# LauraBaracaldo/LauraBaracaldo-Spatial-Meta-Kriging-for-Distributed-Inference-for-Binary-Response

Measured on AMD Instinct MI355X. Metric: MCMC iters/sec (all subsets, whole node) + end-to-end wall-clock, n=500k K=250, higher is better.
Workload: dtype f64

## Files before the change

### laurabaracaldo-spatial-meta-kriging-for-distributed-inference-for-binary-response_amd/csrc/mk_gemm.hpp

```cpp
#pragma once
#include "mk_common.hpp"

namespace mk {

typedef double d4 __attribute__((ext_vector_type(4)));
typedef double d2 __attribute__((ext_vector_type(2)));

constexpr int GB_K = 16;
__host__ __device__ constexpr int gb_stride(int len) {
  return len == 256 ? 272 : (len == 128 ? 144 : (len == 64 ? 80 : 48));
}
__host__ __device__ constexpr int gb_img(int len) { return GB_K * gb_stride(len); }
__host__ __device__ constexpr int gb_lds_bytes(int tm, int tn) { return 2 * (gb_img(tm) + gb_img(tn)) * 8; }
static_assert(gb_lds_bytes(128, 128) == MK_GD_LDS_BYTES, "mk_common.hpp LDS size");
static_assert(128 * GB_K <= gb_img(128) && 64 * GB_K <= gb_img(64) && 32 * GB_K <= gb_img(32),
              "k-contiguous images fit their slots");

template <int BM, int BN>
struct AccT {
  d4 v[BM][BN];
};
typedef AccT<4, 4> Acc;

template <int BM, int BN>
// ... 258 lines not shown
  for (int w = 0; w < 4; ++w) {
    if (syrk_rb(w, 0) != w || syrk_cb(w, SYRK_SLOTS - 1) != 7 - w) return false;
    for (int s = 4; s < SYRK_SLOTS; ++s)
      if (syrk_rb(w, s) != 7 - w) return false;
  }
  return true;
}
static_assert(syrk_rows_static(), "slot 0 / slots 4.. have the same row choice on every wave");

struct AccSyrk {
  d4 v[SYRK_SLOTS];
};
__device__ inline int syrk_wave() { return __builtin_amdgcn_readfirstlane((int)(threadIdx.x >> 6)); }
__device__ inline int syrk_row(int w, int s) { return 16 * syrk_rb(w, s) + (threadIdx.x & 15); }
__device__ inline int syrk_col(int w, int s, int r) { return 16 * syrk_cb(w, s) + ((threadIdx.x & 63) >> 4) + 4 * r; }

__device__ inline void mma_chunk_syrk(const double* Ps, AccSyrk& acc, int w) {
  constexpr int LD = gb_stride(128);
  const int lane = threadIdx.x & 63;
  const int li = lane & 15, lk = lane >> 4;
#pragma unroll
  for (int ks = 0; ks < GB_K / 4; ++ks) {
    const double* row = Ps + (ks * 4 + lk) * LD + li;
    const double p0 = row[16 * w], p1 = row[16 * (7 - w)];
    const double y0 = -p0, y1 = -p1;
    double xb[SYRK_SLOTS];
#pragma unroll
    for (int s = 0; s < SYRK_SLOTS - 1; ++s) xb[s] = row[16 * syrk_cb(w, s)];
    xb[SYRK_SLOTS - 1] = p1;
#pragma unroll
    for (int s = 0; s < SYRK_SLOTS; ++s) {
      const double ya = s == 0 ? y0 : (s >= 4 ? y1 : (s <= w ? y0 : y1));
      acc.v[s] = __builtin_amdgcn_mfma_f64_16x16x4f64(xb[s], ya, acc.v[s], 0, 0, 0);
    }
  }
}

__device__ inline void gemm_syrk_128(const double* __restrict__ P, long s, int K, AccSyrk& acc, double* lds) {
  constexpr int STAGE = gb_img(128);
  if (K <= 0) return;
  const int nch = K / GB_K;
  const int w = syrk_wave();
  dma_chunk<true, 128>(P, s, 0, lds);
  asm volatile("s_waitcnt vmcnt(0)" ::: "memory");
  __syncthreads();
  for (int c = 0; c < nch; ++c) {
    if (c + 1 < nch) dma_chunk<true, 128>(P, s, GB_K * (c + 1), lds + ((c + 1) & 1) * STAGE);
    mma_chunk_syrk(lds + (c & 1) * STAGE, acc, w);
    asm volatile("s_waitcnt vmcnt(0)" ::: "memory");
    __syncthreads();
  }
}

__device__ inline void acc_load_syrk(AccSyrk& acc, const double* C, long ldc) {
  const int w = syrk_wave();
#pragma unroll
  for (int s = 0; s < SYRK_SLOTS; ++s)
#pragma unroll
    for (int r = 0; r < 4; ++r) acc.v[s][r] = C[syrk_row(w, s) + (long)syrk_col(w, s, r) * ldc];
}
__device__ inline void store_tile_syrk(double* C, long ldc, const AccSyrk& acc) {
  const int w = syrk_wave();
#pragma unroll
  for (int s = 0; s < SYRK_SLOTS; ++s)
#pragma unroll
    for (int r = 0; r < 4; ++r) C[syrk_row(w, s) + (long)syrk_col(w, s, r) * ldc] = acc.v[s][r];
}
__device__ inline void store_tile_syrk_lds(double* T, int tld, const AccSyrk& acc) {
  const int w = syrk_wave();
#pragma unroll
  for (int s = 0; s < SYRK_SLOTS; ++s)
#pragma unroll
    for (int r = 0; r < 4; ++r) {
      const int rr = syrk_row(w, s), cc = syrk_col(w, s, r);
      T[rr + cc * tld] = rr >= cc ? acc.v[s][r] : 0.0;
    }
  const int zr = threadIdx.x & 15, zc = threadIdx.x >> 4;
#pragma unroll
  for (int rb = 0; rb < 8; ++rb)
#pragma unroll
    for (int cb = rb + 1; cb < 8; ++cb) T[(16 * rb + zr) + (16 * cb + zc) * tld] = 0.0;
}

}
```

### laurabaracaldo-spatial-meta-kriging-for-distributed-inference-for-binary-response_amd/csrc/mk_kernels.hpp

```cpp
#pragma once
#include "mk_types.hpp"
#include "mk_corr.hpp"

namespace mk {
inline int xcd_grid_h(int S, int T) { return 8 * ((S + 7) / 8) * T; }
template <int MODEL>
__global__ void k_cov_candidate(Model md, MatSet ms, int h0, int hc, int which, int iter, const int* slist, const int* scount);
typedef void (*CovCandidateKernel)(Model, MatSet, int, int, int, int, const int*, const int*);
inline CovCandidateKernel cov_candidate_kernel(int model) {
  return model == MK_COV_EXPONENTIAL ? k_cov_candidate<MK_COV_EXPONENTIAL> : k_cov_candidate<MK_COV_MATERN>;
}
template <int TM, int TN = TM>
__global__ void k_chol_update(MatSet ms, int S, int h0, int hc, int k, int ia, int ib, int j0, int j1,
                              const int* slist, const int* scount, int syrk);
template <int TM>
__global__ void k_chol_trsm(MatSet ms, int S, int h0, int hc, int k, int ia, int ib, const int* slist,
                            const int* scount);
int pv_grid(int max_entries, int nt, int ntt);
template <int TM>
__global__ void k_chol_update_trsm(MatSet ms, int S, int h0, int hc, int k, int ia, int ib, int j0, int extra,
                                   const int* slist, const int* scount, int syrk);
__global__ void k_chol_diag(MatSet ms, const int* n_s, int h0, int hc, int k, double* ld_part, double* quad_c, int* info,
                            const int* slist, const int* scount, int cj0, int cj1, int syrk);
__global__ void k_inv_copydiag(MatSet ms, const int* list, const int* count);
template <int TM>
__global__ void k_inv_level(MatSet ms, const int* list, const int* count, int sz, int phase);
__global__ void k_lauum(MatSet ms, const int* n_s, const int* list, const int* count);
__global__ void k_qblocks(MatSet ms, const int* n_s, const int* list, const int* count);
__global__ void k_take_border(Model md, MatSet ms, const int* list, const int* count, const double* zc);
__global__ void k_cand_border(Model md, MatSet ms, int h0, int hc);
__global__ void k_pred_draw_runs(Model md, const double* kz, const double* kA, int k_lo, const int* plist,
                                 const int* pcount, const int* run_start, int j_end);
__global__ void k_run_start(const int* plist, const int* pcount, int* run_start, int j);
__global__ void k_border_step(Model md, MatSet ms, int k);
__global__ void k_nu_border(Model md, MatSet ms);
__global__ void k_border_quad(Model md);
__global__ void k_trmv_Z(Model md, MatSet ms);
template <int MODEL>
__global__ void k_pred_PT(Model md, const int* list, const int* count);
__global__ void k_pred_PT_matern(Model md, const int* list, const int* count);
__global__ void k_matern_table(Model md, int h0, int hc, int which, int iter, const int* slist, const int* scount);
__global__ void k_matern_table_list(Model md, const int* list, const int* count);
typedef void (*PredPTKernel)(Model, const int*, const int*);
inline PredPTKernel pred_PT_kernel(int model) {
  return model == MK_COV_EXPONENTIAL ? k_pred_PT<MK_COV_EXPONENTIAL> : k_pred_PT<MK_COV_MATERN>;
}
template <bool GEN>
__global__ void k_pred_var(Model md, MatSet ms, const int* list, const int* count);
__global__ void k_pred_var_reduce(Model md, int nt, const int* list, const int* count);
__global__ void k_beta(Model md, int iter);
__global__ void k_Aphase(Model md, int iter);
__global__ void k_theta_mh(Model md, MatSet ms, int h0, int hc, int which, int iter);
__global__ void k_dirty_list(Model md, int force, int* list_inv, int* count_inv, int* list_pred, int* count_pred);
template <int Q>
__global__ void k_sweep(Model md, MatSet ms, int iter, const int* adm, int* fb);
template <int Q>
__global__ void k_sweep_mg(Model md, MatSet ms, int iter, double* part, int* cnt, int* xcc, int* err, int* adm, int spins_max);
template <int Q, int KR, int P, int HH, int LN>
__global__ void k_sweep_site(Model md, MatSet ms, int iter);
inline size_t sweep_site_lds_bytes(int ns_max, int q, int lean = 0) { return (size_t)ns_max * q * (lean ? 4 : 3) * 8 + (size_t)ns_max * 4; }
inline const void* sweep_site_kernel(int q, int kr, int lean = 1) {
  if (q == 1) {
    if (kr == 1)
      return lean == 1 ? (const void*)k_sweep_site<1, 4, 2, 0, 1> : (const void*)k_sweep_site<1, 4, 2, 0, 2>;
    return lean == 1 ? (const void*)k_sweep_site<1, 8, 2, 0, 1> : (const void*)k_sweep_site<1, 8, 2, 0, 2>;
  }
  switch (q) {
    case 2: return kr == 1 ? (const void*)k_sweep_site<2, 4, 1, 0, 0> : (const void*)k_sweep_site<2, 8, 1, 0, 0>;
    case 3: return kr == 1 ? (const void*)k_sweep_site<3, 4, 1, 0, 0> : nullptr;
    default: return nullptr;
  }
}
template <int Q>
__global__ void k_sweep_step(Model md, MatSet ms, int iter, int B, double* part);
inline const void* sweep_step_kernel(int q) {
  switch (q) {
    case 1: return (const void*)k_sweep_step<1>;
    case 2: return (const void*)k_sweep_step<2>;
    case 3: return (const void*)k_sweep_step<3>;
    default: return (const void*)k_sweep_step<4>;
  }
}
inline const void* sweep_kernel(int q, bool mg) {
  switch (q) {
    case 1: return mg ? (const void*)k_sweep_mg<1> : (const void*)k_sweep<1>;
    case 2: return mg ? (const void*)k_sweep_mg<2> : (const void*)k_sweep<2>;
    case 3: return mg ? (const void*)k_sweep_mg<3> : (const void*)k_sweep<3>;
    default: return mg ? (const void*)k_sweep_mg<4> : (const void*)k_sweep<4>;
  }
}
__global__ void k_record(Model md, int iter);
__global__ void k_record_w(Model md, int iter);
__global__ void k_adapt(Model md, int b);
__global__ void k_pred_draw(Model md, int iter, int kidx);
__global__ void k_quantiles(const double* data, long subset_stride, long row_stride, int n_rows, int n_cols,
                            const double* probs, int n_probs, double* out);
__global__ void k_quantiles_prob(const double* data, long subset_stride, long row_stride, int n_rows, int n_cols,
                                 const double* probs, int n_probs, double* out, ProbSrc ps);
__global__ void k_pred_prob(const double* w, long row_stride, int n_rows, int n_cols, double* out, ProbSrc ps);
__global__ void k_chain_diag(const double* data, long subset_stride, long row_stride, int n_rows, int n_cols, double* out);
__global__ void k_chain_diag_prob(const double* data, long subset_stride, long row_stride, int n_rows, int n_cols,
                                  double* out, ProbSrc ps);
__global__ void k_diag_worst(const double* d, int S, long C, double* out);
__global__ void k_combine(const double* grids, int K, long G, double* out, int mean);
__global__ void k_record_kept(Model md, int kidx);
__global__ void k_kept_dirty(Model md, const double* th_prev, int* slist, int* scount, int* plist, int* pcount);
__global__ void k_flip_pairs(MatSet ms, const int* plist, const int* pcount);
__global__ void k_kept_phi(Model md, const double* th, int n, double* phis);
__global__ void k_krig_g(Model md, MatSet ms, const double* z, double* Gt, int j, int nkp);
// ... 21 lines not shown
```

### laurabaracaldo-spatial-meta-kriging-for-distributed-inference-for-binary-response_amd/csrc/mk_linalg.hip

```cpp
#include "mk_gemm.hpp"
#include "mk_types.hpp"
#include "mk_corr.hpp"

namespace mk {

__device__ inline void candidate_theta(const Model& md, int s, int h, int which, int iter, double* phi, double* nu) {
  const Key key = subset_key(md, s);
  const double* th = md.theta + (long)s * md.n_theta;
  const int idx_phi = md.ntri + h, idx_nu = md.ntri + md.q + h;
  double tphi = th[idx_phi];
  double tnu = (md.cov_model == MK_COV_MATERN) ? th[idx_nu] : 0.0;
  if (which == 0 || which == 1) {
    const int j_mh = (which == 0) ? md.o_phi + h : md.o_nu + h;
    const double z = proposal_normal(key, (uint32_t)j_mh, (uint32_t)iter);
    const double step = exp(md.tune[(long)s * md.n_mh_max + j_mh]) * z;
    if (which == 0) tphi += step; else tnu += step;
  }
  *phi = logit_inv(tphi, md.phi_a[h], md.phi_b[h]);
  *nu = (md.cov_model == MK_COV_MATERN) ? logit_inv(tnu, md.nu_a[h], md.nu_b[h]) : 0.0;
}

struct CandGen {
  const double* cx;
  const double* cy;
// ... 744 lines not shown
  if (cj1 > cj0 && syrk) {
    AccSyrk a;
    acc_load_syrk(a, Mt, ld);
    gemm_syrk_128(M + base + (long)cj0 * MK_NB * ld, ld, (cj1 - cj0) * MK_NB, a, sm);
    store_tile_syrk_lds(T, TLD, a);
  } else if (cj1 > cj0) {
    Acc acc;
    acc_load(acc, Mt, ld);
    const long jo = (long)cj0 * MK_NB * ld;
    gemm_tile<128, 128, true, true, true>(M + base + jo, ld, M + base + jo, ld, (cj1 - cj0) * MK_NB,
                                          (cj1 - cj0) * MK_NB, acc, sm);
#pragma unroll
    for (int bm = 0; bm < 4; ++bm)
#pragma unroll
      for (int bn = 0; bn < 4; ++bn)
#pragma unroll
        for (int r = 0; r < 4; ++r) {
          const int rr = acc_row<128>(bm), cc = acc_col<128>(bn, r);
          T[rr + cc * TLD] = rr >= cc ? acc.v[bm][bn][r] : 0.0;
        }
  } else {
    constexpr int NL = MK_NB * MK_NB / (256 * 2);
    d2 v[NL];
#pragma unroll
    for (int j = 0; j < NL; ++j) {
      const int e = 2 * (tid + 256 * j);
      v[j] = *reinterpret_cast<const d2*>(Mt + (e & 127) + (long)(e >> 7) * ld);
    }
#pragma unroll
    for (int j = 0; j < NL; ++j) {
      const int e = 2 * (tid + 256 * j);
      const int r = e & 127, c = e >> 7;
      T[r + c * TLD] = (r >= c) ? v[j].x : 0.0;
      T[r + 1 + c * TLD] = (r + 1 >= c) ? v[j].y : 0.0;
    }
  }
  __syncthreads();
  MK_TSTAMP(40);
  bool bad = false;
  double* W = winv_slot(ms, sh, slot, k);
  factor_invert_tile(T, dg, xd, Sb, ns - base, quad_c + sh, &bad);
  if (tid < 64) {
    double v = 0.0;
    for (int r = tid; r < MK_NB; r += 64) v += (base + r < ns) ? 2.0 * log(dg[r]) : 0.0;
#pragma unroll
    for (int o = 32; o > 0; o >>= 1) v += __shfl_xor(v, o, 64);
    if (tid == 0) {
      ld_part[(long)sh * ms.nt + k] = v;
      if (bad) info[sh] = 1;
    }
  }
  MK_TSTAMP(41);
  store_tile_lw(T, dg, xd, Mt, ld, W);
  MK_TSTAMP(42);
}

#ifndef MK_TRI_SKIP
#define MK_TRI_SKIP 1
#endif
__device__ inline double* wmat(const MatSet& ms, int sh) { return ms.W + (long)sh * mat_elems(ms); }

__global__ __launch_bounds__(256) void k_inv_copydiag(MatSet ms, const int* __restrict__ list, const int* __restrict__ count) {
  const int part = blockIdx.x % MK_CD_SPLIT, rest = blockIdx.x / MK_CD_SPLIT;
  const int e = rest / ms.nt, k = rest % ms.nt;
  if (e >= *count) return;
  const int sh = list[e];
  const double* Wd = winv_slot(ms, sh, ms.cur[sh], k);
  const long ld = ms.ld;
  double* Wt = wmat(ms, sh) + k * MK_NB + (long)k * MK_NB * ld;
  constexpr int PER = MK_NB * MK_NB / MK_CD_SPLIT;
  const int e0 = part * PER;
  d2 v[PER / 512];
#pragma unroll
  for (int j = 0; j < PER / 512; ++j) v[j] = *reinterpret_cast<const d2*>(Wd + e0 + 2 * (threadIdx.x + 256 * j));
#pragma unroll
  for (int j = 0; j < PER / 512; ++j) {
    const int e2 = e0 + 2 * (threadIdx.x + 256 * j);
    *reinterpret_cast<d2*>(Wt + (e2 & 127) + (long)(e2 >> 7) * ld) = v[j];
  }
}

template <int TM>
__global__ __launch_bounds__(256, 2) void k_inv_level(MatSet ms, const int* __restrict__ list,
                                                      const int* __restrict__ count, int sz, int phase) {
  extern __shared__ __attribute__((aligned(16))) double lds[];
  constexpr int SUBR = MK_NB / TM, SUB = SUBR * SUBR;
  const int npairs = (ms.nt + 2 * sz - 1) / (2 * sz);
  const int per = npairs * sz * sz;
  int e, t;
  if (!xcd_map(*count, per * SUB, &e, &t)) return;
  const int st = t % SUB;
  t /= SUB;
  const int sr = st % SUBR, sc = st / SUBR;
  const int p = t / (sz * sz);
  t %= sz * sz;
  const int T0 = 2 * p * sz, B0 = T0 + sz;
  const int i = B0 + (phase == 0 ? t % sz : t / sz), j = T0 + (phase == 0 ? t / sz : t % sz);
  if (i >= ms.nt) return;
  const int sh = list[e];
  const int cur = ms.cur[sh];
  const long ld = ms.ld;
  double* Wm = wmat(ms, sh);
  double* Y = ms.Y ? ms.Y + (long)sh * mat_elems(ms) : mat_slot(ms, sh, 1 - cur);
  const int ro = sr * TM;
  const long co = (long)sc * TM * ld;
  AccT<TM / 32, TM / 32> acc;
  acc_zero(acc);
  if (phase == 0) {
    const double* Lm = mat_slot(ms, sh, cur);
    const int K = (B0 - j) * MK_NB;
    gemm_tile<TM, TM, true, false, false, true, false, MK_TRI_SKIP ? SKIP_TRI_BL : SKIP_NONE>(
        Lm + i * MK_NB + ro + (long)j * MK_NB * ld, ld, Wm + j * MK_NB + (long)j * MK_NB * ld + co, ld, K, K, acc, lds,
        0, ro / 16, sc * TM / 16);
    store_tile(Y + i * MK_NB + ro + (long)j * MK_NB * ld + co, ld, acc);
  } else {
    const int K = (i - B0 + 1) * MK_NB;
    gemm_tile<TM, TM, true, false, true, false, false, MK_TRI_SKIP ? SKIP_TRI_A : SKIP_NONE>(
        Wm + i * MK_NB + ro + (long)B0 * MK_NB * ld, ld, Y + B0 * MK_NB + (long)j * MK_NB * ld + co, ld, K, K, acc, lds,
        K - MK_NB, ro / 16, sc * TM / 16);
    store_tile(Wm + i * MK_NB + ro + (long)j * MK_NB * ld + co, ld, acc);
  }
}
template __global__ void k_inv_level<128>(MatSet, const int*, const int*, int, int);
template __global__ void k_inv_level<64>(MatSet, const int*, const int*, int, int);
template __global__ void k_inv_level<32>(MatSet, const int*, const int*, int, int);

template <bool DIAG>
__device__ inline void wtw_tile(const MatSet& ms, int sh, int ns, int i, int j, Acc& acc, double* lds) {
  const double* X = wmat(ms, sh);
  const long ld = ms.ld;
  const int K = (ms.nt - i) * MK_NB;
  const int kvalid = ns - i * MK_NB;
  acc_zero(acc);
  if (kvalid > 0)
    gemm_128<false, false, false, false, DIAG, SKIP_NONE, true>(X + i * MK_NB + (long)i * MK_NB * ld, ld,
                                               X + i * MK_NB + (long)j * MK_NB * ld, ld, K, kvalid, acc, lds);
}

__global__ __launch_bounds__(256, 2) void k_lauum(MatSet ms, const int* __restrict__ n_s, const int* __restrict__ list,
                                               const int* __restrict__ count) {
  extern __shared__ __attribute__((aligned(16))) double lds[];
  const int ntiles = ms.nt * (ms.nt + 1) / 2;
  const int e = blockIdx.x / ntiles;
  if (e >= *count) return;
  int t = blockIdx.x % ntiles;
  int i = 0;
  while ((i + 1) * (i + 2) / 2 <= t) ++i;
  const int j = t - i * (i + 1) / 2;
  const int sh = list[e];
  Acc acc;
  wtw_tile<false>(ms, sh, n_s[sh / ms.q], i, j, acc, lds);
  const long ld = ms.ld;
  double* Q = ms.Q + (long)sh * mat_elems(ms);
  double* Ct = (i != j) ? Q + j * MK_NB + (long)i * MK_NB * ld : nullptr;
  store_tile(Q + i * MK_NB + (long)j * MK_NB * ld, ld, acc, Ct);
}

__global__ __launch_bounds__(256, 2) void k_qblocks(MatSet ms, const int* __restrict__ n_s, const int* __restrict__ list,
                                                 const int* __restrict__ count) {
  extern __shared__ __attribute__((aligned(16))) double lds[];
  int e, t;
  if (!xcd_map(*count, ms.nt * 2, &e, &t)) return;
  const int i = t >> 1, sd = t & 1;
  const int sh = list[e];
  const int ns = n_s[sh / ms.q];
  const double* X = wmat(ms, sh);
  const long ld = ms.ld;
  const int K = (ms.nt - i) * MK_NB;
  const int kvalid = ns - i * MK_NB;
  AccT<2, 2> acc;
  acc_zero(acc);
  if (kvalid > 0)
    gemm_tile<64, 64, false, false, false, false, true, SKIP_NONE, true>(
        X + i * MK_NB + (long)(i * MK_NB + 64 * sd) * ld, ld, X + i * MK_NB + (long)(i * MK_NB + 64 * sd) * ld, ld,
        K, kvalid, acc, lds);
  store_tile(ms.QB + ((long)sh * ms.nt + i) * MK_NB * MK_NB + 64 * sd + 64 * sd * MK_NB, MK_NB, acc);
}

__global__ __launch_bounds__(256) void k_take_border(Model md, MatSet ms, const int* __restrict__ list,
                                                     const int* __restrict__ count, const double* __restrict__ zc) {
  const int per = (md.n_pad + 255) / 256;
  const int e = blockIdx.x / per;
  if (e >= *count) return;
  const int sh = list[e];
  const int s = sh / md.q, h = sh % md.q;
  const int ns = md.n_s[s];
  const int j = (blockIdx.x % per) * 256 + threadIdx.x;
  if (j >= md.n_pad) return;
  const long zo = ((long)s * md.q + h) * md.n_pad + j;
  if (zc) {
    md.z[zo] = (j < ns) ? zc[zo] : 0.0;
    return;
  }
  const double* M = mat_slot(ms, sh, ms.cur[sh]);
  md.z[zo] = (j < ns) ? M[ns + (long)j * ms.ld] : 0.0;
}

__global__ __launch_bounds__(256) void k_nu_border(Model md, MatSet ms) {
  const int per = (md.n_pad + 255) / 256;
  const int e = blockIdx.x / per;
  if (e >= md.S * md.q || !md.la_nu[e]) return;
  const int s = e / md.q;
  const int ns = md.n_s[s];
  const int j = (blockIdx.x % per) * 256 + threadIdx.x;
  if (j >= md.n_pad) return;
  const double* M = mat_slot(ms, e, ms.cur[e]);
  md.zc[(long)e * md.n_pad + j] = (j < ns) ? M[ns + (long)j * ms.ld] : 0.0;
}
// ... 401 lines not shown
```

### laurabaracaldo-spatial-meta-kriging-for-distributed-inference-for-binary-response_amd/csrc/mk_schedule.hip

```cpp
#include <hip/hip_runtime.h>
#include <algorithm>
#include <cmath>
#include <vector>
#include "mk_gemm.hpp"
#include "mk_session.hpp"

using namespace mk;

void mk::drain_timers(mk_session* s) {
  std::vector<std::pair<float, float>> upd;
  for (auto& t : s->prof.pending) {
    hipEventSynchronize(t.b);
    float ms = 0.f;
    hipEventElapsedTime(&ms, t.a, t.b);
    if (t.cnt >= 0) t.flops *= (double)s->prof.inv_cnt[t.cnt];
    s->prof.stats[t.which].launches += 1;
    s->prof.stats[t.which].ms += ms;
    s->prof.stats[t.which].flops += t.flops;
    if (t.which == KS_CHOL_UPDATE || t.which == KS_CHOL_UPDATE_SUB) {
      float t0 = 0.f;
      hipEventElapsedTime(&t0, s->prof.pending.front().a, t.a);
      upd.push_back({t0, t0 + ms});
      s->prof.stats[KS_UPDATE_BUSY].launches += 1;
      s->prof.stats[KS_UPDATE_BUSY].flops += t.flops;
// ... 4 lines not shown
  for (auto& iv : upd) {
    if (iv.first > hi) {
      if (hi > lo) busy += hi - lo;
      lo = iv.first;
      hi = iv.second;
    } else {
      hi = std::max(hi, (double)iv.second);
    }
  }
  if (hi > lo) busy += hi - lo;
  s->prof.stats[KS_UPDATE_BUSY].ms += busy;
  for (auto& t : s->prof.pending) {
    hipEventDestroy(t.a);
    hipEventDestroy(t.b);
  }
  s->prof.pending.clear();
  s->prof.inv_cnt_used = 0;
}

static constexpr size_t LDS_128 = gb_lds_bytes(128, 128), LDS_64 = gb_lds_bytes(64, 64),
                        LDS_64x128 = gb_lds_bytes(64, 128), LDS_32 = gb_lds_bytes(32, 32),
                        LDS_32x128 = gb_lds_bytes(32, 128);
bool mk::set_gemm_lds() {
  const std::pair<const void*, size_t> fns[] = {
      {(const void*)k_chol_diag, (size_t)MK_DIAG_LDS_BYTES},
      {(const void*)k_chol_update<128>, LDS_128}, {(const void*)k_chol_update<64>, LDS_64},
      {(const void*)k_chol_trsm<128>, LDS_128},   {(const void*)k_chol_trsm<64>, LDS_64x128},
      {(const void*)k_inv_level<128>, LDS_128},   {(const void*)k_inv_level<64>, LDS_64},
      {(const void*)k_chol_update<32>, LDS_32},   {(const void*)k_chol_trsm<32>, LDS_32x128},
      {(const void*)k_chol_update_trsm<128>, LDS_128}, {(const void*)k_chol_update_trsm<64>, LDS_128},
      {(const void*)k_inv_level<32>, LDS_32},
      {(const void*)k_qblocks, LDS_64},           {(const void*)k_lauum, LDS_128},
      {(const void*)k_pred_var<true>, LDS_128},   {(const void*)k_pred_var<false>, LDS_128}};
  for (const auto& f : fns)
    if (hipFuncSetAttribute(f.first, hipFuncAttributeMaxDynamicSharedMemorySize, (int)f.second) != hipSuccess)
      return false;
  return true;
}

int mk::launch_quantiles(unsigned grid, hipStream_t st, const double* data, long subset_stride, long row_stride,
                         int n_rows, int n_cols, const double* probs, int n_probs, double* out) {
  HIPCHK(hipFuncSetAttribute((const void*)k_quantiles, hipFuncAttributeMaxDynamicSharedMemorySize, MK_QUANT_MAX * 8));
  if (n_rows < 1 || n_rows > MK_QUANT_MAX)
    return set_err(MK_E_ARG, "quantile summaries take 1 .. " + std::to_string(MK_QUANT_MAX) + " kept samples");
  size_t n2 = 1;
  while (n2 < (size_t)n_rows) n2 <<= 1;
  MK_LAUNCH(k_quantiles, dim3(grid), dim3(256), n2 * 8, st, data, subset_stride, row_stride, n_rows, n_cols,
                     probs, n_probs, out);
  HIPCHK(hipGetLastError());
  return 0;
}

int mk::launch_quantiles_prob(unsigned grid, hipStream_t st, const double* data, long subset_stride, long row_stride,
                              int n_rows, int n_cols, const double* probs, int n_probs, double* out, const ProbSrc& ps) {
  HIPCHK(hipFuncSetAttribute((const void*)k_quantiles_prob, hipFuncAttributeMaxDynamicSharedMemorySize, MK_QUANT_MAX * 8));
  if (n_rows < 1 || n_rows > MK_QUANT_MAX)
    return set_err(MK_E_ARG, "quantile summaries take 1 .. " + std::to_string(MK_QUANT_MAX) + " kept samples");
  size_t n2 = 1;
  while (n2 < (size_t)n_rows) n2 <<= 1;
  MK_LAUNCH(k_quantiles_prob, dim3(grid), dim3(256), n2 * 8, st, data, subset_stride, row_stride, n_rows, n_cols,
                     probs, n_probs, out, ps);
  HIPCHK(hipGetLastError());
  return 0;
}

static int tile_size(long wg128) {
  static const int force = env_int("MK_TILE", 0);
  if (force == 32 || force == 64 || force == 128) return force;
  return wg128 >= 256 ? 128 : 64;
}

void mk::launch_candidates(const Model& md, const MatSet& ms, hipStream_t st, int n_entries, int h0, int hc, int which,
                           int iter, const int* slist, const int* scount) {
  if (md.cov_model == MK_COV_MATERN && md.chtab)
    MK_LAUNCH(k_matern_table, dim3(n_entries), dim3(256), 0, st, md, h0, hc, which, iter, slist, scount);
  const int ntiles = ms.nt * (ms.nt + 1) / 2;
  MK_LAUNCH(cov_candidate_kernel(md.cov_model), dim3(xcd_grid_h(n_entries, ntiles)),
                     dim3(256), 0, st, md, ms, h0, hc, which, iter, slist, scount);
}


static int diag_syrk() {
  static const int on = env_int("MK_DIAG_SYRK", 1);
  return on != 0;
}

static void chol_update(mk_session* s, Group& g, hipStream_t st, int h0, int hc, int k, int ia, int ib, int j0, int j1,
                        const int* slist, const int* scount, double flops) {
  const int E = g.S * hc, nti = ib - ia;
  if (nti <= 0) return;
  const int tm = tile_size((long)E * nti);
  if (tm == 32) {
    timed(s, st, KS_CHOL_UPDATE_SUB, flops, [&] {
      MK_LAUNCH(k_chol_update<32>, dim3(xcd_grid_h(E, nti * 16)), dim3(256), LDS_32, st, g.ms, g.S, h0, hc, k, ia,
                         ib, j0, j1, slist, scount, diag_syrk());
    });
  } else if (tm == 64) {
    timed(s, st, KS_CHOL_UPDATE_SUB, flops, [&] {
      MK_LAUNCH(k_chol_update<64>, dim3(xcd_grid_h(E, nti * 4)), dim3(256), LDS_64, st, g.ms, g.S, h0, hc, k, ia,
                         ib, j0, j1, slist, scount, diag_syrk());
    });
  } else {
    timed(s, st, KS_CHOL_UPDATE, flops, [&] {
      MK_LAUNCH(k_chol_update<128>, dim3(xcd_grid_h(E, nti)), dim3(256), LDS_128, st, g.ms, g.S, h0, hc, k, ia,
                         ib, j0, j1, slist, scount, diag_syrk());
    });
  }
}
static void chol_trsm(mk_session* s, Group& g, hipStream_t st, int h0, int hc, int k, int ia, int ib, const int* slist,
                      const int* scount, double flops) {
  const int E = g.S * hc, nti = ib - ia;
  if (nti <= 0) return;
  const int tm = tile_size((long)E * nti);
  timed(s, st, KS_CHOL_TRSM, flops, [&] {
    if (tm == 32)
      MK_LAUNCH(k_chol_trsm<32>, dim3(xcd_grid_h(E, nti * 4)), dim3(256), LDS_32x128, st, g.ms, g.S, h0, hc, k,
                         ia, ib, slist, scount);
    else if (tm == 64)
      MK_LAUNCH(k_chol_trsm<64>, dim3(xcd_grid_h(E, nti * 2)), dim3(256), LDS_64x128, st, g.ms, g.S, h0, hc, k,
                         ia, ib, slist, scount);
    else
      MK_LAUNCH(k_chol_trsm<128>, dim3(xcd_grid_h(E, nti)), dim3(256), LDS_128, st, g.ms, g.S, h0, hc, k, ia, ib,
                         slist, scount);
  });
}
static void chol_update_trsm(mk_session* s, Group& g, hipStream_t st, int h0, int hc, int k, int j0, int extra,
                             const int* slist, const int* scount, double flops) {
  const int E = g.S * hc, nt = s->nt, nti = nt - (k + 1);
  const int tm = tile_size((long)E * (nti + extra));
  timed(s, st, tm == 128 ? KS_CHOL_UPDATE : KS_CHOL_UPDATE_SUB, flops, [&] {
    if (tm == 128)
      MK_LAUNCH(k_chol_update_trsm<128>, dim3(xcd_grid_h(E, nti + extra)), dim3(256), LDS_128, st, g.ms, g.S, h0, hc,
                k, k + 1, nt, j0, extra, slist, scount, diag_syrk());
    else
      MK_LAUNCH(k_chol_update_trsm<64>, dim3(xcd_grid_h(E, 2 * nti + extra)), dim3(256), LDS_128, st, g.ms, g.S, h0,
                hc, k, k + 1, nt, j0, extra, slist, scount, diag_syrk());
  });
}
static void chol_diag(mk_session* s, Group& g, hipStream_t st, int h0, int hc, int k, const int* slist,
                      const int* scount, int cj0 = 0, int cj1 = 0, double flops = 0.0) {
  timed(s, st, KS_CHOL_DIAG, flops, [&] {
    MK_LAUNCH(k_chol_diag, dim3(g.S * hc), dim3(256), (size_t)MK_DIAG_LDS_BYTES, st, g.ms, g.md.n_s, h0, hc, k,
                       g.md.ld_part, g.md.quad_c, g.md.info, slist, scount, cj0, cj1, diag_syrk());
  });
}

static double panel_flops(mk_session* s, Group& g, int hc, int k, int ia, int ib, bool trsm, int j0 = 0, int j1 = -1) {
  if (j1 < 0) j1 = k;
  double fl = 0.0;
  for (int i = g.s0; i < g.s0 + g.S; ++i) {
    const double nv = (double)s->n_part[i] + 1.0;
    const double cols = std::fmin((double)MK_NB, std::fmax(0.0, nv - (double)k * MK_NB));
    const double depth = std::fmax(0.0, std::fmin((double)j1 * MK_NB, nv) - (double)j0 * MK_NB);
    const bool diag = ia <= k && k < ib;
    const double lo = (double)(diag ? k + 1 : ia) * MK_NB;
    const double rows = std::fmax(0.0, std::fmin(nv, (double)ib * MK_NB) - lo);
    if (trsm)
      fl += rows * cols * cols;
    else
      fl += 2.0 * rows * cols * depth + (diag ? cols * (cols + 1.0) * depth : 0.0);
  }
  return fl * hc;
}

static double inv_level_flops(int n, int nt, int sz, int phase) {
  double fl = 0.0;
// ... 11 lines not shown
  if (k_hi < 0) k_hi = nt;
  hipStream_t A = crit ? crit : g.stream;
  static const int fused = env_int("MK_CHOL_FUSED", 1);
  if ((slist || !g.bulk) && fused) {
    for (int k = k_lo; k < k_hi; ++k) {
      const int j0 = k >= 2 ? k - 1 : 0;
      chol_diag(s, g, A, h0, hc, k, slist, scount, j0, k, k > 0 ? panel_flops(s, g, hc, k, k, k + 1, false, j0, k) : 0.0);
      if (k == 0 && nt > 1)
        chol_trsm(s, g, A, h0, hc, 0, 1, nt, slist, scount, panel_flops(s, g, hc, 0, 1, nt, true));
      else if (k > 0 && k < nt - 1)
        chol_update_trsm(s, g, A, h0, hc, k, 0, 1, slist, scount,
                         panel_flops(s, g, hc, k, k + 1, nt, false) + panel_flops(s, g, hc, k, k + 1, nt, true) +
                             panel_flops(s, g, hc, k + 1, k + 1, k + 2, false, 0, k));
      if (evP) hipEventRecord(evP[k], A);
    }
    return;
  }
  if (slist || !g.bulk) {
    for (int k = k_lo; k < k_hi; ++k) {
      if (k > 0)
        chol_update(s, g, A, h0, hc, k, k, nt, 0, k, slist, scount, panel_flops(s, g, hc, k, k, nt, false));
      chol_diag(s, g, A, h0, hc, k, slist, scount);
      if (k < nt - 1)
        chol_trsm(s, g, A, h0, hc, k, k + 1, nt, slist, scount, panel_flops(s, g, hc, k, k + 1, nt, true));
      if (evP) hipEventRecord(evP[k], A);
    }
    return;
  }
  static const int depth_env = env_int("MK_CHOL_DEPTH", 2);
  const int d = std::max(1, std::min(depth_env, 4));
  hipStream_t B = g.bulk;
  hipEvent_t* eT = g.ev.data();
  hipEvent_t* eU = g.ev.data() + nt;
  if (k_lo == 0) {
    hipEventRecord(g.ev[2 * nt], A);
    hipStreamWaitEvent(B, g.ev[2 * nt], 0);
  }
  for (int k = k_lo; k < k_hi; ++k) {
    if (k > d) hipStreamWaitEvent(A, eU[k], 0);
    if (k >= 1) {
      const int j0 = std::max(0, k - d);
      chol_update(s, g, A, h0, hc, k, k, nt, j0, k, nullptr, nullptr, panel_flops(s, g, hc, k, k, nt, false, j0, k));
    }
    chol_diag(s, g, A, h0, hc, k, nullptr, nullptr);
    if (k < nt - 1)
      chol_trsm(s, g, A, h0, hc, k, k + 1, nt, nullptr, nullptr, panel_flops(s, g, hc, k, k + 1, nt, true));
    if (evP) hipEventRecord(evP[k], A);
    if (k + d + 1 < nt) {
      const int c = k + d + 1;
      hipEventRecord(eT[k], A);
      hipStreamWaitEvent(B, eT[k], 0);
      chol_update(s, g, B, h0, hc, c, c, nt, 0, c - d, nullptr, nullptr, panel_flops(s, g, hc, c, c, nt, false, 0, c - d));
      hipEventRecord(eU[c], B);
    }
  }
}

void mk::launch_trinv(mk_session* s, Group& g, int max_entries, const int* list, const int* count) {
  const int nt = s->nt;
  MK_LAUNCH(k_inv_copydiag, dim3(max_entries * nt * MK_CD_SPLIT), dim3(256), 0, g.stream, g.ms, list, count);
  int cnt = -1;
  if (s->prof.on && s->prof.iter && ((s->prof.kinds >> KS_INV) & 1u)) {
    if (!s->prof.inv_cnt && hipHostMalloc((void**)&s->prof.inv_cnt, Profiler::INV_CNT_CAP * sizeof(int)) != hipSuccess) {
      (void)hipGetLastError();
      s->prof.inv_cnt = nullptr;
    }
    if (s->prof.inv_cnt && s->prof.inv_cnt_used < Profiler::INV_CNT_CAP) {
      cnt = s->prof.inv_cnt_used++;
      hipMemcpyAsync(s->prof.inv_cnt + cnt, count, sizeof(int), hipMemcpyDeviceToHost, g.stream);
    }
  }
  for (int sz = 1; sz < nt; sz *= 2) {
    const int npairs = (nt + 2 * sz - 1) / (2 * sz);
    const int tm = tile_size((long)max_entries * npairs * sz * sz / 8);
    for (int phase = 0; phase < 2; ++phase) {
      double per = 0.0;
      if (cnt >= 0) {
        for (int i = g.s0; i < g.s0 + g.S; ++i) per += inv_level_flops(s->n_part[i], nt, sz, phase);
        per /= std::max(1, g.S);
      }
      auto launch = [&] {
        if (tm == 32)
          MK_LAUNCH(k_inv_level<32>, dim3(xcd_grid_h(max_entries, npairs * sz * sz * 16)), dim3(256), LDS_32,
                             g.stream, g.ms, list, count, sz, phase);
        else if (tm == 64)
          MK_LAUNCH(k_inv_level<64>, dim3(xcd_grid_h(max_entries, npairs * sz * sz * 4)), dim3(256), LDS_64,
                             g.stream, g.ms, list, count, sz, phase);
        else
          MK_LAUNCH(k_inv_level<128>, dim3(xcd_grid_h(max_entries, npairs * sz * sz)), dim3(256), LDS_128,
                             g.stream, g.ms, list, count, sz, phase);
      };
      if (cnt >= 0)
        timed(s, g.stream, KS_INV, per, launch, cnt);
      else
        launch();
    }
  }
}

void mk::launch_inverse(mk_session* s, Group& g, bool from_zc) {
  const int nt = s->nt, max_entries = g.S * s->q;
  launch_trinv(s, g, max_entries, g.d_list, g.d_count);
  if (!s->sweep.site)
    timed(s, g.stream, KS_LAUUM, 0.0, [&] {
      MK_LAUNCH(k_qblocks, dim3(xcd_grid_h(max_entries, nt * 2)), dim3(256), LDS_64, g.stream, g.ms, g.md.n_s,
                g.d_list, g.d_count);
    });
  MK_LAUNCH(k_take_border, dim3(max_entries * ((s->n_pad + 255) / 256)), dim3(256), 0, g.stream, g.md, g.ms,
                     g.d_list, g.d_count, from_zc ? (const double*)g.md.zc : nullptr);
}

static double pred_flops(mk_session* s, Group& g) {
  double fl = 0.0;
  for (int i = g.s0; i < g.s0 + g.S; ++i) fl += (double)s->n_part[i] * s->n_part[i] * g.md.n_test;
  return fl * s->q;
}

void mk::launch_pred_refresh(mk_session* s, Group& g, hipStream_t st) {
  Model& md = g.md;
  if (md.n_test <= 0) return;
  if (!st) st = g.stream;
  const int nt = s->nt, max_entries = g.S * s->q;
  if (md.cov_model == MK_COV_MATERN && md.chtab_p)
    MK_LAUNCH(k_matern_table_list, dim3(max_entries), dim3(256), 0, st, md, g.d_plist, g.d_pcount);
  if (md.cov_model == MK_COV_MATERN)
    MK_LAUNCH(k_pred_PT_matern, dim3(max_entries * (md.n_pad / MK_PT_RB)), dim3(256), 0, st, md, g.d_plist,
                       g.d_pcount);
  else if (!s->pred_gen)
    MK_LAUNCH(pred_PT_kernel(md.cov_model), dim3(max_entries * md.n_pad), dim3(256), 0, st, md, g.d_plist,
                       g.d_pcount);
  timed(s, st, KS_PRED_VAR, pred_flops(s, g), [&] {
    MK_LAUNCH(s->pred_gen ? k_pred_var<true> : k_pred_var<false>, dim3(pv_grid(max_entries, nt, md.ntt)),
              dim3(256), LDS_128, st, md, g.ms, g.d_plist, g.d_pcount);
  });
  MK_LAUNCH(k_pred_var_reduce, dim3(max_entries * (md.n_test_pad / 256)), dim3(256), 0, st, md, nt,
                     g.d_plist, g.d_pcount);
}

bool mk::la_auto(const mk_session* s) { return (long)s->S * s->q <= 224; }

static bool use_sweep_mg(const mk_session* s) { return s->sweep.coop; }

static void launch_sweep(mk_session* s, Group& g, int it) {
  const int q = s->q;
  Model md = g.md;
  MatSet ms = g.ms;
  int iter = it;
  hipError_t e = hipSuccess;
  if (s->sweep.site) {
    void* args[] = {&md, &ms, &iter};
    e = hipLaunchKernel(sweep_site_kernel(q, s->sweep.site, s->sweep.lean), dim3(g.S), dim3(MK_SS_T), args,
                        s->sweep.site_lds, g.stream);
    wd_trace(g.stream, "k_sweep_site");
  } else if (use_sweep_mg(s)) {
    hipMemsetAsync(s->sweep.sw_cnt, 0, (size_t)s->S * (s->n_pad / 64 + 1) * sizeof(int), g.stream);
    double* part = s->sweep.sw_part;
    int* cnt = s->sweep.sw_cnt;
    int* xcc = s->sweep.sw_xcc;
    int* err = s->sweep.sw_err;
    int* adm = s->sweep.sw_adm;
    int spins = s->sweep.adm_spins;
    void* args[] = {&md, &ms, &iter, &part, &cnt, &xcc, &err, &adm, &spins};
    e = hipLaunchKernel(sweep_kernel(q, true), dim3(xcd_grid(g.S, s->nt)), dim3(256), args, s->sweep.mg_lds,
                        g.stream);
    wd_trace(g.stream, "k_sweep_mg");
    if (e == hipSuccess) {
      const size_t sw_lds = (size_t)q * (64 * 64 + 2 * 64) * sizeof(double);
      const int* cadm = adm;
      int* fb = s->sweep.sw_err + 1;
      void* fa[] = {&md, &ms, &iter, &cadm, &fb};
      e = hipLaunchKernel(sweep_kernel(q, false), dim3(g.S), dim3(MK_SW_T), fa, sw_lds, g.stream);
      wd_trace(g.stream, "k_sweep(fallback)");
    }
// ... 199 lines not shown
```

Before: 12430.

## Skip structurally zero triangular MFMA work in 128-tile inverse level GEMMs

```diff
diff --git a/laurabaracaldo-spatial-meta-kriging-for-distributed-inference-for-binary-response_amd/csrc/mk_gemm.hpp b/laurabaracaldo-spatial-meta-kriging-for-distributed-inference-for-binary-response_amd/csrc/mk_gemm.hpp
--- a/laurabaracaldo-spatial-meta-kriging-for-distributed-inference-for-binary-response_amd/csrc/mk_gemm.hpp
+++ b/laurabaracaldo-spatial-meta-kriging-for-distributed-inference-for-binary-response_amd/csrc/mk_gemm.hpp
@@ -364,4 +364,129 @@
     for (int cb = rb + 1; cb < 8; ++cb) T[(16 * rb + zr) + (16 * cb + zc) * tld] = 0.0;
 }
 
-}
+template <bool COL>
+using AccDeal = AccT<COL ? 8 : 2, COL ? 2 : 8>;
+__host__ __device__ constexpr int deal_blk(int w, int d) { return d == 0 ? w : 7 - w; }
+__host__ __device__ constexpr bool deal_live(bool col, int blk, int cp) { return col ? blk <= cp : blk >= cp; }
+__host__ __device__ constexpr bool deal_always(bool col, int d, int cp) {
+  return deal_live(col, col ? 4 * d + 3 : 4 * d, cp);
+}
+__host__ __device__ constexpr bool deal_never(bool col, int d, int cp) {
+  return !deal_live(col, col ? 4 * d : 4 * d + 3, cp);
+}
+constexpr bool deal_cover_exact(bool col) {
+  int cnt[8][8] = {};
+  for (int w = 0; w < 4; ++w) {
+    int mine = 0;
+    for (int cp = 0; cp < 8; ++cp) {
+      int branches = 0;
+      for (int d = 0; d < 2; ++d) {
+        const int blk = deal_blk(w, d);
+        const bool live = deal_live(col, blk, cp);
+        if (deal_always(col, d, cp) && !live) return false;
+        if (deal_never(col, d, cp) && live) return false;
+        if (deal_always(col, d, cp) && deal_never(col, d, cp)) return false;
+        if (!deal_always(col, d, cp) && !deal_never(col, d, cp)) ++branches;
+        if (live) {
+          ++cnt[blk][cp];
+          ++mine;
+        }
+      }
+      if (branches > 1) return false;
+    }
+    if (mine != 9) return false;
+  }
+  for (int blk = 0; blk < 8; ++blk)
+    for (int cp = 0; cp < 8; ++cp)
+      if (cnt[blk][cp] != (deal_live(col, blk, cp) ? 1 : 0)) return false;
+  return true;
+}
+static_assert(deal_cover_exact(false) && deal_cover_exact(true),
+              "both deals cover the live (block, chunk) pairs exactly once, nine per wave");
+
+template <bool COL>
+__device__ inline int deal_row(int w, int bm) { return 16 * (COL ? bm : deal_blk(w, bm)) + (threadIdx.x & 15); }
+template <bool COL>
+__device__ inline int deal_col(int w, int bn, int r) {
+  return 16 * (COL ? deal_blk(w, bn) : bn) + ((threadIdx.x & 63) >> 4) + 4 * r;
+}
+
+template <bool COL, bool NEG, int CP>
+__device__ inline void mma_chunk_deal(const double* As, const double* Bs, AccDeal<COL>& acc, int w) {
+  constexpr int BM = COL ? 8 : 2, BN = COL ? 2 : 8;
+  const int lane = threadIdx.x & 63;
+  const int li = lane & 15, lk = lane >> 4;
+#pragma unroll
+  for (int ks = 0; ks < GB_K / 4; ++ks) {
+    const int k = ks * 4 + lk;
+    double ya[BM], xb[BN];
+#pragma unroll
+    for (int b = 0; b < BM; ++b) {
+      const double av = frag<true, 128>(As, 16 * (COL ? b : deal_blk(w, b)) + li, k);
+      ya[b] = NEG ? -av : av;
+    }
+#pragma unroll
+    for (int b = 0; b < BN; ++b) xb[b] = frag<false, 128>(Bs, 16 * (COL ? deal_blk(w, b) : b) + li, k);
+#pragma unroll
+    for (int d = 0; d < 2; ++d) {
+      if (CP >= 0 && deal_never(COL, d, CP)) continue;
+      if (CP >= 0 && !deal_always(COL, d, CP) && !deal_live(COL, deal_blk(w, d), CP)) continue;
+#pragma unroll
+      for (int o = 0; o < 8; ++o) {
+        if constexpr (COL)
+          acc.v[o][d] = __builtin_amdgcn_mfma_f64_16x16x4f64(xb[d], ya[o], acc.v[o][d], 0, 0, 0);
+        else
+          acc.v[d][o] = __builtin_amdgcn_mfma_f64_16x16x4f64(xb[o], ya[d], acc.v[d][o], 0, 0, 0);
+      }
+    }
+  }
+}
+
+template <bool COL, bool NEG>
+__device__ inline void gemm_deal_128(const double* __restrict__ A, long sA, const double* __restrict__ B, long sB, int K,
+                                     AccDeal<COL>& acc, double* lds) {
+  constexpr bool REV = COL;
+  constexpr int IMG = gb_img(128), STAGE = 2 * IMG;
+  const int nch = K / GB_K, nd = nch - 128 / GB_K;
+  const int w = syrk_wave();
+  auto k_of = [&](int c) { return REV ? K - GB_K * (c + 1) : GB_K * c; };
+  auto issue = [&](int c) {
+    double* st = lds + (c & 1) * STAGE;
+    dma_chunk<true, 128>(A, sA, k_of(c), st);
+    dma_chunk<false, 128>(B, sB, k_of(c), st + IMG);
+  };
+  issue(0);
+  asm volatile("s_waitcnt vmcnt(0)" ::: "memory");
+  __syncthreads();
+  for (int c = 0; c < nd; ++c) {
+    const double* st = lds + (c & 1) * STAGE;
+    issue(c + 1);
+    mma_chunk_deal<COL, NEG, -1>(st, st + IMG, acc, w);
+    asm volatile("s_waitcnt vmcnt(0)" ::: "memory");
+    __syncthreads();
+  }
+#define MK_DEAL_TRI(t)                                                              \
+  {                                                                                 \
+    const double* st = lds + ((t) & 1) * STAGE;                                     \
+    if ((t) < 7) issue(nd + (t) + 1);                                               \
+    mma_chunk_deal<COL, NEG, REV ? 7 - (t) : (t)>(st, st + IMG, acc, w);            \
+    asm volatile("s_waitcnt vmcnt(0)" ::: "memory");                                \
+    __syncthreads();                                                                \
+  }
+  MK_DEAL_TRI(0) MK_DEAL_TRI(1) MK_DEAL_TRI(2) MK_DEAL_TRI(3)
+  MK_DEAL_TRI(4) MK_DEAL_TRI(5) MK_DEAL_TRI(6) MK_DEAL_TRI(7)
+#undef MK_DEAL_TRI
+}
+
+template <bool COL>
+__device__ inline void store_tile_deal(double* C, long ldc, const AccDeal<COL>& acc) {
+  const int w = syrk_wave();
+#pragma unroll
+  for (int bm = 0; bm < (COL ? 8 : 2); ++bm)
+#pragma unroll
+    for (int bn = 0; bn < (COL ? 2 : 8); ++bn)
+#pragma unroll
+      for (int r = 0; r < 4; ++r) C[deal_row<COL>(w, bm) + (long)deal_col<COL>(w, bn, r) * ldc] = acc.v[bm][bn][r];
+}
+
+}
diff --git a/laurabaracaldo-spatial-meta-kriging-for-distributed-inference-for-binary-response_amd/csrc/mk_kernels.hpp b/laurabaracaldo-spatial-meta-kriging-for-distributed-inference-for-binary-response_amd/csrc/mk_kernels.hpp
--- a/laurabaracaldo-spatial-meta-kriging-for-distributed-inference-for-binary-response_amd/csrc/mk_kernels.hpp
+++ b/laurabaracaldo-spatial-meta-kriging-for-distributed-inference-for-binary-response_amd/csrc/mk_kernels.hpp
@@ -24,7 +24,7 @@
                             const int* slist, const int* scount, int cj0, int cj1, int syrk);
 __global__ void k_inv_copydiag(MatSet ms, const int* list, const int* count);
 template <int TM>
-__global__ void k_inv_level(MatSet ms, const int* list, const int* count, int sz, int phase);
+__global__ void k_inv_level(MatSet ms, const int* list, const int* count, int sz, int phase, int deal);
 __global__ void k_lauum(MatSet ms, const int* n_s, const int* list, const int* count);
 __global__ void k_qblocks(MatSet ms, const int* n_s, const int* list, const int* count);
 __global__ void k_take_border(Model md, MatSet ms, const int* list, const int* count, const double* zc);
diff --git a/laurabaracaldo-spatial-meta-kriging-for-distributed-inference-for-binary-response_amd/csrc/mk_linalg.hip b/laurabaracaldo-spatial-meta-kriging-for-distributed-inference-for-binary-response_amd/csrc/mk_linalg.hip
--- a/laurabaracaldo-spatial-meta-kriging-for-distributed-inference-for-binary-response_amd/csrc/mk_linalg.hip
+++ b/laurabaracaldo-spatial-meta-kriging-for-distributed-inference-for-binary-response_amd/csrc/mk_linalg.hip
@@ -850,7 +850,7 @@
 
 template <int TM>
 __global__ __launch_bounds__(256, 2) void k_inv_level(MatSet ms, const int* __restrict__ list,
-                                                      const int* __restrict__ count, int sz, int phase) {
+                                                      const int* __restrict__ count, int sz, int phase, int deal) {
   extern __shared__ __attribute__((aligned(16))) double lds[];
   constexpr int SUBR = MK_NB / TM, SUB = SUBR * SUBR;
   const int npairs = (ms.nt + 2 * sz - 1) / (2 * sz);
@@ -872,6 +872,25 @@
   double* Y = ms.Y ? ms.Y + (long)sh * mat_elems(ms) : mat_slot(ms, sh, 1 - cur);
   const int ro = sr * TM;
   const long co = (long)sc * TM * ld;
+  if constexpr (TM == 128) {
+    if (deal) {
+      if (phase == 0) {
+        const double* Lm = mat_slot(ms, sh, cur);
+        AccDeal<true> acc;
+        acc_zero(acc);
+        gemm_deal_128<true, false>(Lm + i * MK_NB + (long)j * MK_NB * ld, ld, Wm + j * MK_NB + (long)j * MK_NB * ld, ld,
+                                   (B0 - j) * MK_NB, acc, lds);
+        store_tile_deal<true>(Y + i * MK_NB + (long)j * MK_NB * ld, ld, acc);
+      } else {
+        AccDeal<false> acc;
+        acc_zero(acc);
+        gemm_deal_128<false, true>(Wm + i * MK_NB + (long)B0 * MK_NB * ld, ld, Y + B0 * MK_NB + (long)j * MK_NB * ld, ld,
+                                   (i - B0 + 1) * MK_NB, acc, lds);
+        store_tile_deal<false>(Wm + i * MK_NB + (long)j * MK_NB * ld, ld, acc);
+      }
+      return;
+    }
+  }
   AccT<TM / 32, TM / 32> acc;
   acc_zero(acc);
   if (phase == 0) {
@@ -889,9 +908,9 @@
     store_tile(Wm + i * MK_NB + ro + (long)j * MK_NB * ld + co, ld, acc);
   }
 }
-template __global__ void k_inv_level<128>(MatSet, const int*, const int*, int, int);
-template __global__ void k_inv_level<64>(MatSet, const int*, const int*, int, int);
-template __global__ void k_inv_level<32>(MatSet, const int*, const int*, int, int);
+template __global__ void k_inv_level<128>(MatSet, const int*, const int*, int, int, int);
+template __global__ void k_inv_level<64>(MatSet, const int*, const int*, int, int, int);
+template __global__ void k_inv_level<32>(MatSet, const int*, const int*, int, int, int);
 
 template <bool DIAG>
 __device__ inline void wtw_tile(const MatSet& ms, int sh, int ns, int i, int j, Acc& acc, double* lds) {
diff --git a/laurabaracaldo-spatial-meta-kriging-for-distributed-inference-for-binary-response_amd/csrc/mk_schedule.hip b/laurabaracaldo-spatial-meta-kriging-for-distributed-inference-for-binary-response_amd/csrc/mk_schedule.hip
--- a/laurabaracaldo-spatial-meta-kriging-for-distributed-inference-for-binary-response_amd/csrc/mk_schedule.hip
+++ b/laurabaracaldo-spatial-meta-kriging-for-distributed-inference-for-binary-response_amd/csrc/mk_schedule.hip
@@ -110,6 +110,11 @@
 
 static int diag_syrk() {
   static const int on = env_int("MK_DIAG_SYRK", 1);
+  return on != 0;
+}
+
+static int inv_deal() {
+  static const int on = env_int("MK_INV_DEAL", 1);
   return on != 0;
 }
 
@@ -287,13 +292,13 @@
       auto launch = [&] {
         if (tm == 32)
           MK_LAUNCH(k_inv_level<32>, dim3(xcd_grid_h(max_entries, npairs * sz * sz * 16)), dim3(256), LDS_32,
-                             g.stream, g.ms, list, count, sz, phase);
+                             g.stream, g.ms, list, count, sz, phase, inv_deal());
         else if (tm == 64)
           MK_LAUNCH(k_inv_level<64>, dim3(xcd_grid_h(max_entries, npairs * sz * sz * 4)), dim3(256), LDS_64,
-                             g.stream, g.ms, list, count, sz, phase);
+                             g.stream, g.ms, list, count, sz, phase, inv_deal());
         else
           MK_LAUNCH(k_inv_level<128>, dim3(xcd_grid_h(max_entries, npairs * sz * sz)), dim3(256), LDS_128,
-                             g.stream, g.ms, list, count, sz, phase);
+                             g.stream, g.ms, list, count, sz, phase, inv_deal());
       };
       if (cnt >= 0)
         timed(s, g.stream, KS_INV, per, launch, cnt);
```

Result: faster. 12620 (median of 6 runs) (+1.5%).
